# MisterPup/PDE-MultiGrid

Hardware: AMD Instinct MI355X
Metric: MLUPS on 3D Poisson 512^3 V-cycle (higher is better)
Workload: dtype f64

## Files before the change

include/mgx.h:

```cpp
#ifndef MGX_H
#define MGX_H

#include <stddef.h>
#include <stdint.h>

#ifdef __cplusplus
extern "C" {
#endif

typedef enum {
    MGX_OK = 0,
    MGX_ERR_INVALID = 1,
    MGX_ERR_SIZE = 2,
    MGX_ERR_HIP = 3,
    MGX_ERR_NOMEM = 4,
    MGX_ERR_RCCL = 5,
    MGX_ERR_NOGPU = 6
} mgx_status;

typedef enum { MGX_RESIDUAL_REF_COMPAT = 0, MGX_RESIDUAL_CORRECT = 1 } mgx_residual_mode;

typedef struct mgx_ctx mgx_ctx;
typedef struct mgx_event mgx_event;

// ... 6 lines not shown
int mgx_ctx_create(int device, mgx_ctx** out);
int mgx_ctx_destroy(mgx_ctx* ctx);
int mgx_ctx_sync(mgx_ctx* ctx);
int mgx_ctx_check(mgx_ctx* ctx);
int mgx_ctx_clear_abort(mgx_ctx* ctx, int reenable);
int mgx_ctx_generation(const mgx_ctx* ctx, unsigned long long* generation);
int mgx_ctx_prepare(mgx_ctx* ctx);
int mgx_ctx_device(const mgx_ctx* ctx, int* device);
int mgx_ctx_set_param(mgx_ctx* ctx, const char* name, int value);
const char* mgx_ctx_last_relax_kernel(const mgx_ctx* ctx);
const char* mgx_ctx_last_rr_kernel(const mgx_ctx* ctx);
const char* mgx_ctx_last_corr_kernel(const mgx_ctx* ctx);
const char* mgx_ctx_last_block3_kernel(const mgx_ctx* ctx);
int mgx3dxs_relax_block3_f64(mgx_ctx* ctx, const double* vin, double* vout, const double* f, const int n[3], const double h[3],
                             int first_colour, int store_both);
int mgx_test_set_lds_poison(int on);
int mgx_test_lds_probe(mgx_ctx* ctx, double* fraction);
int mgx_ctx_stream(const mgx_ctx* ctx, void** hip_stream);

int mgx_malloc(mgx_ctx* ctx, size_t bytes, void** dptr);
int mgx_free(mgx_ctx* ctx, void* dptr);
int mgx_memcpy_h2d(mgx_ctx* ctx, void* dst, const void* host_src, size_t bytes);
int mgx_memcpy_d2h(mgx_ctx* ctx, void* host_dst, const void* src, size_t bytes);
int mgx_memcpy_d2d(mgx_ctx* ctx, void* dst, const void* src, size_t bytes);
int mgx_memset_zero(mgx_ctx* ctx, void* dst, size_t bytes);

int mgx_graph_begin(mgx_ctx* ctx);
int mgx_graph_end(mgx_ctx* ctx, void** graph_exec);
int mgx_graph_launch(mgx_ctx* ctx, void* graph_exec);
int mgx_graph_destroy(mgx_ctx* ctx, void* graph_exec);
// ... 195 lines not shown
     \
     \
     \
     \
     \
     \
     \
     \
     \
     \
    int mgx3dxs_corr_fused_takes_##SFX(const mgx_ctx* ctx, const int n[3], int nplanes);                \
     \
     \
     \
    int mgx3dxs_block3_up_takes_##SFX(const mgx_ctx* ctx, const int n[3], int ncycles);                 \
    int mgx3dxs_correct_pset_slab_##SFX(mgx_ctx* ctx, real* v, const int n[3], int fzoff,               \
                                        const real* coarse_v, const int cn[3], int czoff, int zmin,     \
                                        int zmax);                                                      \
    int mgx3dxs_relax_corr_colour_slab_##SFX(mgx_ctx* ctx, real* v, const real* f, const int n[3],      \
                                             int fzoff, const real h[3], const real* coarse_v,          \
                                             const int cn[3], int czoff, int cplanes, int zbeg,         \
                                             int zend);                                                 \
     \
     \
     \
    int mgx3dxs_interpolate_correct_colour_##SFX(mgx_ctx* ctx, real* v, const int n[3],                 \
                                                 const real* coarse_v, const int cn[3], int colour);    \
    int mgx3dxs_interpolate_correct_colour_slab_##SFX(mgx_ctx* ctx, real* v, const int n[3], int fzoff, \
                                                      const real* coarse_v, const int cn[3], int czoff, \
                                                      int pzbeg, int pzend, int colour);                \
// ... 203 lines not shown
```

pde_multigrid_amd/csrc/host/mg_multigrid3d.inc:

```

#define GRID MG_CAT(mgGrid3D_, R)
#define MGRID MG_CAT(mgMultiGrid3D_, R)
#define FN(name) MG_CAT3(mgMultiGrid3D_, R, _##name)
#define MGXL(mg, name) ((mg)->layout ? MG_CAT3(mgx3dxs_, name##_, R) : MG_CAT3(mgx3d_, name##_, R))

static size_t MG_CAT(vol3_, R)(const GRID* g) { return (size_t)g->sizeX * g->sizeY * g->sizeZ; }
static size_t MG_CAT(dvol3_, R)(int layout, const GRID* g) {
    return layout ? MG_CAT(mgx3dxs_elems_, R)(g->sizeXYZ) : MG_CAT(vol3_, R)(g);
}

static int MG_CAT(grid3_new_, R)(mgx_ctx* ctx, int layout, const int sizeXYZ[3], const REAL range[6], GRID** out) {
    for (int d = 0; d < 3; d++)
        MG_REQUIRE(sizeXYZ[d] >= 3 && (sizeXYZ[d] - 1) % 2 == 0, MGX_ERR_SIZE, "Grid3D: size[%d] = %d is not odd and >= 3", d,
                   sizeXYZ[d]);
    MG_REQUIRE(range[1] > range[0] && range[3] > range[2] && range[5] > range[4], MGX_ERR_INVALID,
               "Grid3D: empty range");
    GRID* g = (GRID*)calloc(1, sizeof(GRID));
    MG_REQUIRE(g, MGX_ERR_NOMEM, "Grid3D: out of host memory");
    g->sizeX = g->sizeXYZ[0] = sizeXYZ[0];
    g->sizeY = g->sizeXYZ[1] = sizeXYZ[1];
    g->sizeZ = g->sizeXYZ[2] = sizeXYZ[2];
    REAL x_range = range[1] - range[0];
    REAL y_range = range[3] - range[2];
    REAL z_range = range[5] - range[4];
// ... 523 lines not shown
        if (down_done) {
        } else if (mg->fuse && mg->f_rim_zero[gridID + 1]) {
            MG_TRY(MGXL(mg, residual_restrict_keep_rim)(mg->ctx, fine->d_v, fine->d_f, fine->sizeXYZ, h, mg->residual_mode,
                                                        coarse->d_f, coarse->sizeXYZ));
        } else if (mg->fuse) {
            MG_TRY(MGXL(mg, residual_restrict)(mg->ctx, fine->d_v, fine->d_f, fine->sizeXYZ, h, mg->residual_mode, coarse->d_f,
                                          coarse->sizeXYZ));
            mg->f_rim_zero[gridID + 1] = 1;
        } else {
            REAL* residual = NULL;
            MG_TRY(FN(CalculateResidual)(mg, fine, &residual));
            MG_TRY(FN(Restrict)(mg, residual, fine->sizeXYZ, coarse->d_f, coarse->sizeXYZ));
        }
        MG_TRY(MG_CAT(vcycle_body3_, R)(mg, gridID + 1, v1, v2, 1));
        if (mg->fuse && mg->layout && mg->smoother == 0 && v2 > 0) {
            MG_TRY(MG_CAT(mgx3dxs_interpolate_correct_relax_pp_, R)(mg->ctx, fine->d_v, fine->d_e, fine->d_f, fine->sizeXYZ, h, coarse->d_v,
                                                                    coarse->sizeXYZ, v2, mg->e_rim_valid[gridID]));
            if (MG_CAT(mgx3dxs_relax_pp_takes_, R)(mg->ctx, fine->sizeXYZ, v2) && !MG_CAT(mgx3dxs_corr_fused_takes_, R)(mg->ctx, fine->sizeXYZ, fine->sizeZ - 2))
                mg->e_rim_valid[gridID] = 1;
            if (MG_CAT(mgx3dxs_block3_up_takes_, R)(mg->ctx, fine->sizeXYZ, v2))
                mg->e_rim_valid[gridID] = 1;
            return MGX_OK;
        } else if (mg->fuse) {
            MG_TRY(MGXL(mg, interpolate_correct)(mg->ctx, fine->d_v, fine->sizeXYZ, coarse->d_v, coarse->sizeXYZ));
        } else {
            MG_TRY(FN(Interpolate)(mg, fine->d_e, fine->sizeXYZ, coarse->d_v, coarse->sizeXYZ));
            MG_TRY(FN(ApplyCorrection)(mg, fine->d_v, fine->sizeXYZ, fine->d_e, fine->sizeXYZ));
        }
    }
    return FN(Relax)(mg, fine, v2);
// ... 370 lines not shown
```

pde_multigrid_amd/csrc/mgx_block3d.hip:

```cpp
#include <type_traits>

#include "mgx_internal.hpp"
#include "mgx_kernels3d.hpp"

namespace mgx {

template <class real, int COL, bool STORE_BOTH, int TW>
__global__ void __launch_bounds__(64 * TW, 4)
    relax3d_xs_block3_kernel(const real* vin, real* vout, const real* __restrict__ f, int sx, int sy, int sz, real hx2, real hy2,
                             real hz2, int zrun, int gx, int gy, int xcd_mode) {
    constexpr int ROWS = 2 * TW, OUTR = ROWS - 6;
    static_assert(OUTR % 2 == 0, "the colour parity of a wave's rows must not depend on the tile");
    __shared__ real sY[2][TW][2][64];
    __shared__ real sX[2][TW][2][64];
    __shared__ real sZ[2][TW][2][64];
    const Geo<XSplit, real> g(sx, sy);
    const int lane = threadIdx.x;
    const int w = __builtin_amdgcn_readfirstlane(threadIdx.y);
    int bx, by, bz;
    tile_of_block(xcd_mode, gx, gy, bx, by, bz);
    const int z0 = 1 + bz * zrun, z1 = min(z0 + zrun, sz - 1);
    if (z0 >= z1) return;
    const int PL = (int)g.PL;

    const int Hn = (sx + 1) >> 1;
    const int pn = bx * 60 + lane - 2, p = min(max(pn, 0), Hn - 1);
    const unsigned off0 = (unsigned)p * (unsigned)sizeof(real), off1 = (unsigned)(g.H + (p <= Hn - 2 ? p : 0)) * (unsigned)sizeof(real);
// ... 3 lines not shown
    const bool xface0 = pn <= 0 || pn >= Hn - 1;
    const bool wxface = bx * 60 - 2 <= 0 || bx * 60 + 61 >= Hn - 1;
    const bool outlane = lane >= 2 && lane <= 61;
    int roff[2];
    bool yin[2], outrow[2];
#pragma unroll
    for (int o = 0; o < 2; o++) {
        const int y = by * OUTR - 3 + 2 * w + o;
        roff[o] = min(max(y, 0), sy - 1) * g.P;
        yin[o] = y >= 1 && y <= sy - 2;
        outrow[o] = 2 * w + o >= 3 && 2 * w + o < ROWS - 3;
    }
    const int wU = w > 0 ? w - 1 : 0, wD = w < TW - 1 ? w + 1 : TW - 1;
    auto zc = [&](int z) { return min(max(z, 0), sz - 1); };
    auto plane = [&](const real* a, int z) { return plane_rsrc<real>(a + (ptrdiff_t)zc(z) * (ptrdiff_t)g.PL, PL, 1); };

    real a_m[2], a_c[2], a_p[2], a_n[2], fx_c[2], fx_1[2], fx_2[2], fx_n[2], xv_n[2], fy_c[2], fy_n[2];
    real b_c[2], b_m[2], b_mm[2], d_c[2], d_m[2], d_mm[2], x3[2];
#pragma unroll
    for (int o = 0; o < 2; o++)
        a_m[o] = a_c[o] = a_p[o] = a_n[o] = fx_c[o] = fx_1[o] = fx_2[o] = fx_n[o] = xv_n[o] = fy_c[o] = fy_n[o] = b_c[o] =
            b_m[o] = b_mm[o] = d_c[o] = d_m[o] = d_mm[o] = x3[o] = 0;

    const int t0 = z0 - 2, tlast = z1 + 1;
    {
        const auto qm = plane(vin, t0 - 1), q0 = plane(vin, t0), qp = plane(vin, t0 + 1);
        const bool zf = t0 <= 0 || t0 >= sz - 1;
        const auto qf = plane(f, t0);
#pragma unroll
        for (int o = 0; o < 2; o++) {
            const int hx = (COL + 1 + o + t0) & 1;
            a_m[o] = buf_load<real>(qm, off(hx), roff[o]);
            a_c[o] = buf_load<real>(q0, off(hx ^ 1), roff[o]);
            a_p[o] = buf_load<real>(qp, off(hx), roff[o]);
            fx_c[o] = buf_load<real>(zf || !yin[o] ? q0 : qf, off(hx), roff[o]);
            if (wxface) xv_n[o] = buf_load<real>(q0, off(0), roff[o]);
        }
        __builtin_amdgcn_s_waitcnt(0x0F70);
#pragma unroll
        for (int o = 0; o < 2; o++)
            if (wxface && ((COL + 1 + o + t0) & 1) == 0 && xface0) fx_c[o] = xv_n[o];
        const int b = (t0 - 1) & 1;
        sY[b][w][0][lane] = a_c[0];
        sY[b][w][1][lane] = a_c[1];
        asm volatile("s_waitcnt lgkmcnt(0)\n\ts_barrier" ::: "memory");
    }

    auto relax = [&](auto hc, int o, const real (&c)[2], real nb, real sb, real D, real U, real fv) __attribute__((always_inline)) {
        constexpr int h = decltype(hc)::value;
        real O, E;
        if (h == 0) {
            O = wave_from_prev_lane<real>(c[o]);
            E = c[o];
        } else {
            O = c[o];
            E = wave_from_next_lane<real>(c[o]);
// ... 8 lines not shown
        const auto ro3 = plane(vout, t - 3), ro2 = plane(vout, t - 2);
        const auto rY = plane(vin, t + 2), rXv = plane(vin, t + 1), rFx = plane(f, t + 1), rFy = plane(f, t);
        const bool zf = t + 1 <= 0 || t + 1 >= sz - 1;
        __builtin_amdgcn_s_setprio(3);
#pragma unroll
        for (int o = 0; o < 2; o++) {
            const int hx = (COL + 1 + o + PAR) & 1;
            const bool sto = outlane && yin[o] && outrow[o];
            if (t - 3 >= z0 && t - 3 < z1 && sto && xin(hx ^ 1)) buf_store_nt<real>(x3[o], ro3, off(hx ^ 1), roff[o]);
            if (STORE_BOTH && t - 2 >= z0 && t - 2 < z1 && sto && xin(hx ^ 1)) buf_store_nt<real>(d_m[o], ro2, off(hx ^ 1), roff[o]);
            a_n[o] = buf_load<real>(rY, off(hx ^ 1), roff[o]);
            fx_n[o] = buf_load<real>(zf || !yin[o] ? rXv : rFx, off(hx ^ 1), roff[o]);
            if ((hx ^ 1) == 0 && wxface) xv_n[o] = buf_load<real>(rXv, off(0), roff[o]);
            fy_n[o] = buf_load<real>(rFy, off(hx ^ 1), roff[o]);
        }
        __builtin_amdgcn_s_setprio(0);
        const bool zin1 = t >= 1 && t <= sz - 2, zin2 = t - 1 >= 1 && t - 1 <= sz - 2;
        {
            const real nb = sY[PB][wU][1][lane], sb = sY[PB][wD][0][lane];
#pragma unroll
            for (int o = 0; o < 2; o++) {
                const real v1 = (((COL + 1 + PAR) & 1) ^ o) == 0
                                    ? relax(std::integral_constant<int, 0>{}, o, a_c, nb, sb, a_m[o], a_p[o], fx_c[o])
                                    : relax(std::integral_constant<int, 1>{}, o, a_c, nb, sb, a_m[o], a_p[o], fx_c[o]);
                const int hx = (COL + 1 + o + PAR) & 1;
                b_c[o] = zin1 && yin[o] && xin(hx) ? v1 : fx_c[o];
            }
        }
        {
            const real nb = sX[PB][wU][1][lane], sb = sX[PB][wD][0][lane];
// ... 3 lines not shown
                                    ? relax(std::integral_constant<int, 0>{}, o, b_m, nb, sb, b_mm[o], b_c[o], fy_c[o])
                                    : relax(std::integral_constant<int, 1>{}, o, b_m, nb, sb, b_mm[o], b_c[o], fy_c[o]);
                const int hx = (COL + 1 + o + PAR) & 1;
                d_c[o] = zin2 && yin[o] && xin(hx) ? v2 : a_m[o];
            }
        }
        {
            const real nb = sZ[PB][wU][1][lane], sb = sZ[PB][wD][0][lane];
#pragma unroll
            for (int o = 0; o < 2; o++) {
                x3[o] = (((COL + 1 + PAR) & 1) ^ o) == 0
                            ? relax(std::integral_constant<int, 0>{}, o, d_m, nb, sb, d_mm[o], d_c[o], fx_2[o])
                            : relax(std::integral_constant<int, 1>{}, o, d_m, nb, sb, d_mm[o], d_c[o], fx_2[o]);
            }
        }
#pragma unroll
        for (int o = 0; o < 2; o++) {
            sY[PAR][w][o][lane] = a_p[o];
            sX[PAR][w][o][lane] = b_c[o];
            sZ[PAR][w][o][lane] = d_c[o];
        }
        asm volatile("s_waitcnt lgkmcnt(0)\n\ts_barrier" ::: "memory");
        __builtin_amdgcn_s_waitcnt(0x0F70);
#pragma unroll
        for (int o = 0; o < 2; o++) {
            a_m[o] = a_c[o]; a_c[o] = a_p[o]; a_p[o] = a_n[o];
            fx_2[o] = fx_1[o]; fx_1[o] = fx_c[o];
            fx_c[o] = ((COL + 1 + o + PAR) & 1) == 1 && wxface && xface0 ? xv_n[o] : fx_n[o];
            fy_c[o] = fy_n[o];
            b_mm[o] = b_m[o]; b_m[o] = b_c[o];
            d_mm[o] = d_m[o]; d_m[o] = d_c[o];
        }
    };

    int t = t0;
    if (t & 1) iteration(std::integral_constant<int, 1>{}, t++);
    for (;; t += 2) {
        iteration(std::integral_constant<int, 0>{}, t);
        if (t == tlast) break;
        iteration(std::integral_constant<int, 1>{}, t + 1);
        if (t + 1 == tlast) break;
// ... 4 lines not shown
        for (int o = 0; o < 2; o++) {
            const int hx = (COL + 1 + o + tlast) & 1;
            if (outlane && yin[o] && outrow[o] && xin(hx)) buf_store_nt<real>(x3[o], ro3, off(hx), roff[o]);
        }
    }
}

bool relax_block3_takes(const mgx_ctx* ctx, const int n[3], size_t elem, int part) {
    if (!(ctx->block3 & part) || elem != 8) return false;
    if ((unsigned long long)Geo<XSplit, double>(n[0], n[1]).PL * 8ull >= (1ull << 31)) return false;
    return n[0] >= 385 && n[1] >= 129 && n[2] >= 65;
}

template <class real>
void relax3d_xs_block3_launch(mgx_ctx* ctx, const real* vin, real* vout, const real* f, const int n[3], real hx2, real hy2, real hz2,
                              int first_colour, bool store_both) {
    constexpr int TW = 16;
    const int gx = ceil_div((n[0] - 1) / 2, 60), gy = ceil_div(n[1] - 2, 2 * TW - 6);
    const int tiles = gx * gy, planes = n[2] - 2;
    const int zrun = ceil_div(planes, runs_filling_rounds(tiles, planes, ctx->num_cus, 64, 16, 4));
    const dim3 grid(tiles * ceil_div(planes, zrun), 1, 1), blk(64, TW, 1);
#define MGX_B3(C, S)                                                                                                          \
    MGX_LAUNCH((relax3d_xs_block3_kernel<real, C, S, TW>), grid, blk, 0, ctx->compute, vin, vout, f, n[0], n[1], n[2], hx2, hy2, \
               hz2, zrun, gx, gy, 1)
    if (first_colour == 0) {
        if (store_both) MGX_B3(0, true); else MGX_B3(0, false);
    } else {
        if (store_both) MGX_B3(1, true); else MGX_B3(1, false);
    }
#undef MGX_B3
    snprintf(ctx->last_block3_kernel, sizeof ctx->last_block3_kernel, "relax3d_xs_block3_kernel<%s,%d,%s,%d>",
             sizeof(real) == 8 ? "double" : "float", first_colour, store_both ? "true" : "false", TW);
}
template void relax3d_xs_block3_launch<double>(mgx_ctx*, const double*, double*, const double*, const int[3], double, double, double, int,
                                               bool);

}

extern "C" int mgx3dxs_relax_block3_f64(mgx_ctx* ctx, const double* vin, double* vout, const double* f, const int n[3], const double h[3],
                                        int first_colour, int store_both) {
    MGX_REQUIRE(ctx && vin && vout && f && n && h, MGX_ERR_INVALID, "relax_block3: NULL argument");
    MGX_USE(ctx);
    MGX_REQUIRE(mgx::valid_size(n[0]) && mgx::valid_size(n[1]) && mgx::valid_size(n[2]), MGX_ERR_SIZE,
                "relax_block3: sizes %d x %d x %d are not odd and >= 3", n[0], n[1], n[2]);
    MGX_REQUIRE(first_colour == 0 || first_colour == 1, MGX_ERR_INVALID, "relax_block3: first_colour = %d not in {0, 1}", first_colour);
    const unsigned long long plane_bytes = (unsigned long long)mgx::Geo<mgx::XSplit, double>(n[0], n[1]).PL * 8ull;
    MGX_REQUIRE(plane_bytes < (1ull << 31), MGX_ERR_SIZE,
                "relax_block3: a plane of %d x %d is too large", n[0], n[1]);
    MGX_REQUIRE(!store_both || vin != vout, MGX_ERR_INVALID, "relax_block3: store_both needs vout != vin");
    mgx::relax3d_xs_block3_launch<double>(ctx, vin, vout, f, n, h[0] * h[0], h[1] * h[1], h[2] * h[2], first_colour, store_both != 0);
    MGX_LAUNCH_CHECK();
    return MGX_OK;
}
```

pde_multigrid_amd/csrc/mgx_internal.hpp:

```cpp
#pragma once
#include <hip/hip_runtime.h>

#include <cstdarg>
#include <cstdio>
#include <cstring>
#include <type_traits>

#include "mgx.h"

struct mgx_ctx {
    int device = 0;
    hipStream_t compute = nullptr;
    hipStream_t comm = nullptr;
    hipEvent_t ev_compute = nullptr;
    hipEvent_t ev_comm = nullptr;
    int comm_inline = 0;
    int relax_ty = 4;
    int relax_zchunk = 0;
    int relax_xcd = 1;
    int rr_rows = 0;
    int rr_rcp = 1;
    int mixed_fused = 0;
    int mixed_rows = 4;
    int mixed_zchunk = 0;
// ... 37 lines not shown
    size_t scratch_bytes = 0;
    void* rccl_comm = nullptr;
    void* local_group = nullptr;
    int rank = 0, nranks = 1;
    int comm_rehearse = 0;
    void* rehearse_buf = nullptr;
    size_t rehearse_bytes = 0;
    int num_cus = 256;
    int pipe_unroll = 7;
    int corr_low = 0;
    int slab_edges_merged = 1;
    int resident_tile = 0;
    char last_corr_kernel[96] = "";
    char last_rr_kernel[96] = "";
    char last_relax_kernel[96] = "";
    int block3 = 3;
    char last_block3_kernel[96] = "";
};

struct mgx_event {
    hipEvent_t ev = nullptr;
};

namespace mgx {

void set_error(const char* fmt, ...);

inline int fail(int status, const char* fmt, ...) {
    char buf[512];
    va_list ap;
    va_start(ap, fmt);
// ... 82 lines not shown
```

pde_multigrid_amd/csrc/mgx_kernels3d.hip:

```cpp
#include <type_traits>

#include "mgx_internal.hpp"
#include "mgx_kernels3d.hpp"
#include "mgx_sync.hpp"

namespace mgx {

template <class real>
__global__ void __launch_bounds__(256) relax3d_colour_kernel(real* __restrict__ v, const real* __restrict__ f, int sx,
                                                             int sy, int sz, real hx2, real hy2, real hz2, int colour) {
    const int y = 1 + blockIdx.y * blockDim.y + threadIdx.y;
    const int z = 1 + blockIdx.z;
    if (y >= sy - 1) return;
    const int p = (colour + y + z) & 1;
    const int x = 2 * (blockIdx.x * blockDim.x + threadIdx.x) + p;
    if (x < 1 || x >= sx - 1) return;
    const size_t sxy = (size_t)sx * sy;
    const size_t i = x + (size_t)y * sx + (size_t)z * sxy;
    const real O = v[i - 1], E = v[i + 1];
    const real N = v[i - sx], S = v[i + sx];
    const real D = v[i - sxy], U = v[i + sxy];
    v[i] = relax3d_point<real>(O, E, N, S, D, U, f[i], hx2, hy2, hz2);
}

// ... 2559 lines not shown

template <class real, class L>
int residual_restrict3d(mgx_ctx* ctx, const real* v, const real* f, const int n[3], const real h[3], int mode,
                        real* coarse_f, const int cn[3], bool rim_is_zero = false) {
    MGX_TRY_RET(check_rr_args(ctx, ctx && v && f && h && coarse_f, n, cn, "residual_restrict3d"));
    MGX_REQUIRE(mode == MGX_RESIDUAL_REF_COMPAT || mode == MGX_RESIDUAL_CORRECT, MGX_ERR_INVALID,
                "residual_restrict3d: bad mode %d", mode);
    return residual_restrict3d_range<real, L>(ctx, v, f, n, 0, h, mode, coarse_f, cn, 0, 0, cn[2], rim_is_zero);
}

bool relax_rr3d_xs_takes(const mgx_ctx* ctx, const int n[3], const int cn[3], size_t elem);

bool relax_block3_takes(const mgx_ctx* ctx, const int n[3], size_t elem, int part);
template <class real>
void relax3d_xs_block3_launch(mgx_ctx* ctx, const real* vin, real* vout, const real* f, const int n[3], real hx2, real hy2, real hz2,
                              int first_colour, bool store_both);
template <>
void relax3d_xs_block3_launch<float>(mgx_ctx*, const float*, float*, const float*, const int[3], float, float, float, int, bool) {}

template <class real>
int relax_rr3d_slab(mgx_ctx* ctx, real* v, const real* f, const int n[3], int fzoff, const real h[3], int mode, real* coarse_f,
                    const int cn[3], int czoff, int pzbeg, int pzend) {
    MGX_TRY_RET(check_rr_args(ctx, ctx && v && f && h && coarse_f, n, cn, "relax_rr_slab"));
    MGX_REQUIRE(mode == MGX_RESIDUAL_REF_COMPAT || mode == MGX_RESIDUAL_CORRECT, MGX_ERR_INVALID, "relax_rr_slab: bad mode %d", mode);
    MGX_REQUIRE(pzbeg >= 1 && pzend <= cn[2] - 1 && pzbeg < pzend && czoff >= 0 && czoff <= pzbeg && fzoff >= 0 && (fzoff & 1) == 0 &&
                    fzoff <= (2 * pzbeg - 3 > 0 ? 2 * pzbeg - 3 : 0),
                MGX_ERR_INVALID, "relax_rr_slab: coarse planes [%d, %d) with offsets %d / %d", pzbeg, pzend, fzoff, czoff);
    MGX_REQUIRE(relax_rr3d_xs_takes(ctx, n, cn, sizeof(real)), MGX_ERR_INVALID, "relax_rr_slab: the level is not taken (ask relax_rr_takes)");
    const Geo<XSplit, real> gc(cn[0], cn[1]);
    MGX_TRY_RET(fill_zero(ctx, coarse_f + gc.PL * (size_t)(pzbeg - czoff), gc.PL * (size_t)(pzend - pzbeg) * sizeof(real)));
    MGX_REQUIRE(relax_rr3d_xs_launch<real>(ctx, v, f, n, h, mode, coarse_f, cn, fzoff, czoff, pzbeg, pzend), MGX_ERR_INVALID,
                "relax_rr_slab: launch refused");
    MGX_LAUNCH_CHECK();
// ... 221 lines not shown
        pipe_launch<real, false, 2, 4, 2, 2>(ctx, p, v, vo, f, sx, sy, zb, ze, hx2, hy2, hz2, colour, coarse_sh, cx, cy, szl, ckmax, zg0);
    else
        pipe_launch<real, false, 2, 8, 2, 2>(ctx, p, v, vo, f, sx, sy, zb, ze, hx2, hy2, hz2, colour, coarse_sh, cx, cy, szl, ckmax, zg0);
    memcpy(ctx->last_corr_kernel, ctx->last_relax_kernel, sizeof ctx->last_corr_kernel);
}

template <class real>
int relax3d_xs_pp(mgx_ctx* ctx, real* v, real* w, const real* f, const int n[3], const real h[3], int ncycles, int w_rim_valid);
template <class real>
void copy_rim3d_xs(mgx_ctx* ctx, const real* v, real* w, const int n[3]);

static bool block3_up_takes(const mgx_ctx* ctx, const int n[3], size_t elem, int ncycles) {
    return ncycles >= 2 && corr_fused_takes(ctx, n[0], n[1], n[2], n[2] - 2) && relax_block3_takes(ctx, n, elem, 2);
}

template <class real>
int interpolate_correct_relax3d_xs(mgx_ctx* ctx, real* v, const real* f, const int n[3], const real h[3], const real* coarse_v,
                                   const int cn[3], int ncycles, real* w = nullptr, int w_rim_valid = 0) {
    MGX_REQUIRE(ctx && v && f && h && coarse_v, MGX_ERR_INVALID, "interpolate_correct_relax3d: NULL argument");
    MGX_USE(ctx);
    int st = check_n3(n, "interpolate_correct_relax3d");
    if (st) return st;
    st = check_coarse3(n, cn, "interpolate_correct_relax3d");
    if (st) return st;
    MGX_REQUIRE(ncycles >= 1, MGX_ERR_INVALID, "interpolate_correct_relax3d: ncycles = %d < 1 (use interpolate_correct)", ncycles);
    ctx->last_corr_kernel[0] = 0;
    ctx->last_block3_kernel[0] = 0;
    const real hx2 = h[0] * h[0], hy2 = h[1] * h[1], hz2 = h[2] * h[2];
    const int sx = n[0], sy = n[1], sz = n[2], zb = 1, ze = sz - 1;
    if (!corr_fused_takes(ctx, sx, sy, sz, ze - zb)) {
        st = interpolate_correct3d_slab<real>(ctx, v, n, 0, coarse_v, cn, 0, 0, cn[2] - 1, 1);
        if (st) return st;
        if (w) return relax3d_xs_pp<real>(ctx, v, w, f, n, h, ncycles, w_rim_valid);
// ... 296 lines not shown
                                                        coarse_f, cn, coarse_rim_is_zero);                       \
    }                                                                                                            \
    int mgx3dxs_relax_rr_takes_##SFX(const mgx_ctx* ctx, const int n[3], const int cn[3]) {                     \
        return ctx && n && cn && mgx::relax_rr3d_xs_takes(ctx, n, cn, sizeof(real));                             \
    }                                                                                                            \
    int mgx3dxs_relax_rr_slab_##SFX(mgx_ctx* ctx, real* v, const real* f, const int n[3], int fzoff,            \
                                    const real h[3], int mode, real* coarse_f, const int cn[3], int czoff,       \
                                    int pzbeg, int pzend) {                                                      \
        return mgx::relax_rr3d_slab<real>(ctx, v, f, n, fzoff, h, mode, coarse_f, cn, czoff, pzbeg, pzend);      \
    }                                                                                                            \
    int mgx3dxs_corr_fused_takes_##SFX(const mgx_ctx* ctx, const int n[3], int nplanes) {                        \
        return ctx && n && mgx::corr_fused_takes(ctx, n[0], n[1], n[2], nplanes);                                \
    }                                                                                                            \
    int mgx3dxs_block3_up_takes_##SFX(const mgx_ctx* ctx, const int n[3], int ncycles) {                         \
        return ctx && n && mgx::block3_up_takes(ctx, n, sizeof(real), ncycles);                                  \
    }                                                                                                            \
    int mgx3dxs_correct_pset_slab_##SFX(mgx_ctx* ctx, real* v, const int n[3], int fzoff, const real* coarse_v,  \
                                        const int cn[3], int czoff, int zmin, int zmax) {                        \
        return mgx::correct_pset3d_slab<real>(ctx, v, n, fzoff, coarse_v, cn, czoff, zmin, zmax);                \
    }                                                                                                            \
    int mgx3dxs_relax_corr_colour_slab_##SFX(mgx_ctx* ctx, real* v, const real* f, const int n[3], int fzoff,    \
                                             const real h[3], const real* coarse_v, const int cn[3], int czoff,  \
                                             int cplanes, int zbeg, int zend) {                                  \
        return mgx::relax3d_corr_colour_slab<real>(ctx, v, f, n, fzoff, h, coarse_v, cn, czoff, cplanes, zbeg,   \
                                                   zend);                                                        \
    }                                                                                                            \
    int mgx3dxs_interpolate_correct_relax_pp_##SFX(mgx_ctx* ctx, real* v, real* w, const real* f, const int n[3], \
                                                   const real h[3], const real* coarse_v, const int cn[3],       \
                                                   int ncycles, int w_rim_valid) {                               \
        if (!w) return mgx::fail(MGX_ERR_INVALID, "interpolate_correct_relax_pp: w is NULL");                    \
// ... 154 lines not shown
#else
        return mgx::fail(MGX_ERR_INVALID, "set_param: 'relax3d.fused_dbg' exists only in diagnostic builds (make diag)");
#endif
    } else if (!strcmp(name, "relax3d.fused_lead")) {
        MGX_REQUIRE(value == 0 || (value >= 5 && value <= 7), MGX_ERR_INVALID, "relax3d.fused_lead (planes the red stage runs ahead) must be 0 (default), 5, 6 or 7");
        ctx->sweep_lead = value;
    } else if (!strcmp(name, "relax3d.unroll")) {
        MGX_REQUIRE(value >= 0 && value <= 31, MGX_ERR_INVALID, "set_param: relax3d.unroll = %d not in [0, 31]", value);
        ctx->pipe_unroll = value;
    } else if (!strcmp(name, "relax3d.block3")) {
        MGX_REQUIRE(value == 0 || value == 1, MGX_ERR_INVALID, "set_param: relax3d.block3 = %d not in {0, 1}", value);
        ctx->block3 = (ctx->block3 & ~1) | value;
    } else if (!strcmp(name, "relax3d.block3_up")) {
        MGX_REQUIRE(value == 0 || value == 1, MGX_ERR_INVALID, "set_param: relax3d.block3_up = %d not in {0, 1}", value);
        ctx->block3 = (ctx->block3 & ~2) | (value << 1);
    } else if (!strcmp(name, "relax3d.zchunk")) {
        MGX_REQUIRE(value >= 0, MGX_ERR_INVALID, "relax3d.zchunk must be >= 0 (0 = automatic)");
        ctx->relax_zchunk = value;
    } else {
        return mgx::fail(MGX_ERR_INVALID, "set_param: unknown parameter '%s'", name);
    }
    return MGX_OK;
}
}
```

pde_multigrid_amd/multigrid.py:

```python
import ctypes as C

import numpy as np

from ._lib import CORRECT, REF_COMPAT, check, lib


def _ct(dtype):
    dtype = np.dtype(dtype)
    if dtype == np.float32:
        return "f32", C.c_float
    if dtype == np.float64:
        return "f64", C.c_double
    raise TypeError("dtype must be float32 or float64, got %s" % dtype)


def _ip(a):
    return (C.c_int * len(a))(*[int(x) for x in a])


def _rp(a, ct):
    return (ct * len(a))(*[float(x) for x in a])


def _shape(n):
# ... 262 lines not shown

    def sweep_once(self, ctx, vin, vout, f, n, rng, zero=False, dtype=None):
        dtype = dtype or vin.dtype
        fn, ct = self._fn("sweep_once", dtype)
        h = _rp(grid_spacing(n, rng, dtype), ct)
        return self._run(ctx, [vin, vout, f], lambda a, o, b: fn(ctx._h, a, o, b, _ip(n), h, C.c_int(int(zero))), 1, _shape(n), dtype)

    def relax_pp_takes(self, ctx, n, ncycles, dtype=np.float64):
        s, _ = _ct(dtype)
        return bool(getattr(lib, "mgx3dxs_relax_pp_takes_" + s)(ctx._h, _ip(n), C.c_int(ncycles)))

    def block3_up_takes(self, ctx, n, ncycles, dtype=np.float64):
        s, _ = _ct(dtype)
        return bool(getattr(lib, "mgx3dxs_block3_up_takes_" + s)(ctx._h, _ip(n), C.c_int(ncycles)))

    def residual(self, ctx, v, f, n, rng, mode=REF_COMPAT, dtype=None):
        dtype = dtype or v.dtype
        fn, ct = self._fn("residual", dtype)
        h = _rp(grid_spacing(n, rng, dtype), ct)
        r = np.zeros(_shape(n), dtype)
        return self._run(ctx, [v, f, r], lambda a, b, c: fn(ctx._h, a, b, c, _ip(n), h, C.c_int(mode)), 2, _shape(n), dtype)

    def residual_restrict(self, ctx, v, f, n, rng, mode=REF_COMPAT, dtype=None):
        dtype = dtype or v.dtype
        fn, ct = self._fn("residual_restrict", dtype)
        h = _rp(grid_spacing(n, rng, dtype), ct)
        cn = coarse_size(n)
        coarse = np.zeros(_shape(cn), dtype)
        return self._run(ctx, [v, f, coarse], lambda a, b, c: fn(ctx._h, a, b, _ip(n), h, C.c_int(mode), c, _ip(cn)), 2,
                         _shape(cn), dtype)
# ... 55 lines not shown
            out_v = xs_unpack(ctx.to_host(pv, tuple(_shape(n)[:-1]) + (xs_geometry(n[0], isz)[1],), dtype), n[0])
            out_c = xs_unpack(ctx.to_host(pc, tuple(_shape(cn)[:-1]) + (xs_geometry(cn[0], isz)[1],), dtype), cn[0])
            return out_v, out_c
        finally:
            for q in (pv, pf, pc):
                ctx.free(q)

    def relax_block3(self, ctx, vin, f, n, rng, first_colour=0, store_both=False, vout=None):
        h = _rp(grid_spacing(n, rng, np.float64), C.c_double)
        arrs = [vin, f] if vout is None else [vin, f, vout]
        if vout is None:
            call = lambda a, b: lib.mgx3dxs_relax_block3_f64(ctx._h, a, a, b, _ip(n), h, C.c_int(first_colour), C.c_int(int(store_both)))
            return self._run(ctx, arrs, call, 0, _shape(n), np.float64)
        call = lambda a, b, c: lib.mgx3dxs_relax_block3_f64(ctx._h, a, c, b, _ip(n), h, C.c_int(first_colour), C.c_int(int(store_both)))
        return self._run(ctx, arrs, call, 2, _shape(n), np.float64)

    def interpolate_correct_relax(self, ctx, v, f, n, rng, coarse, ncycles, dtype=None):
        dtype = dtype or v.dtype
        fn, ct = self._fn("interpolate_correct_relax", dtype)
        h = _rp(grid_spacing(n, rng, dtype), ct)
        cn = coarse_size(n)
        return self._run(ctx, [v, f, coarse], lambda a, b, c: fn(ctx._h, a, b, _ip(n), h, c, _ip(cn), C.c_int(ncycles)), 0, _shape(n),
                         dtype)

    def jacobi(self, ctx, v, f, n, rng, omega, ncycles, dtype=None):
        dtype = dtype or v.dtype
        fn, ct = self._fn("jacobi", dtype)
        h = _rp(grid_spacing(n, rng, dtype), ct)
        return self._run(ctx, [v, np.zeros_like(v), f], lambda a, t, b: fn(ctx._h, a, t, b, _ip(n), h, ct(omega), C.c_int(ncycles)),
                         0, _shape(n), dtype)
# ... 922 lines not shown
```

Before: 226,900.

## Fuse coarse-grid interpolation correction into the block3 three-colour relax kernel

Adds a CORR variant of the temporally blocked block3 relax kernel that streams coarse-grid planes, trilinearly interpolates the correction on the fly, and adds it to the fine values as they enter the register pipeline. The post-smoothing path then uses this kernel, followed by remaining single passes, instead of a separate interpolate-correct-relax sequence. The block3_corr bit is enabled by default. This removes a full pass over the fine grid for the correction. In exchange the kernel carries more registers and extra coarse loads, which may reduce occupancy.

```diff
diff --git a/include/mgx.h b/include/mgx.h
--- a/include/mgx.h
+++ b/include/mgx.h
@@ -44,6 +44,8 @@
 const char* mgx_ctx_last_block3_kernel(const mgx_ctx* ctx);
 int mgx3dxs_relax_block3_f64(mgx_ctx* ctx, const double* vin, double* vout, const double* f, const int n[3], const double h[3],
                              int first_colour, int store_both);
+int mgx3dxs_relax_block3_corr_f64(mgx_ctx* ctx, double* v, const double* f, const int n[3], const double h[3], const double* coarse_v,
+                                  const int cn[3]);
 int mgx_test_set_lds_poison(int on);
 int mgx_test_lds_probe(mgx_ctx* ctx, double* fraction);
 int mgx_ctx_stream(const mgx_ctx* ctx, void** hip_stream);
@@ -269,6 +271,15 @@
      \
      \
     int mgx3dxs_block3_up_takes_##SFX(const mgx_ctx* ctx, const int n[3], int ncycles);                 \
+     \
+     \
+     \
+     \
+    int mgx3dxs_block3_corr_takes_##SFX(const mgx_ctx* ctx, const int n[3], int ncycles);               \
+    int mgx3dxs_interpolate_correct_relax_block3_##SFX(mgx_ctx* ctx, real* v, const real* f,            \
+                                                       const int n[3], const real h[3],                 \
+                                                       const real* coarse_v, const int cn[3],           \
+                                                       int ncycles);                                    \
     int mgx3dxs_correct_pset_slab_##SFX(mgx_ctx* ctx, real* v, const int n[3], int fzoff,               \
                                         const real* coarse_v, const int cn[3], int czoff, int zmin,     \
                                         int zmax);                                                      \
diff --git a/pde_multigrid_amd/csrc/host/mg_multigrid3d.inc b/pde_multigrid_amd/csrc/host/mg_multigrid3d.inc
--- a/pde_multigrid_amd/csrc/host/mg_multigrid3d.inc
+++ b/pde_multigrid_amd/csrc/host/mg_multigrid3d.inc
@@ -561,6 +561,11 @@
         }
         MG_TRY(MG_CAT(vcycle_body3_, R)(mg, gridID + 1, v1, v2, 1));
         if (mg->fuse && mg->layout && mg->smoother == 0 && v2 > 0) {
+            if (MG_CAT(mgx3dxs_block3_corr_takes_, R)(mg->ctx, fine->sizeXYZ, v2)) {
+                MG_TRY(MG_CAT(mgx3dxs_interpolate_correct_relax_block3_, R)(mg->ctx, fine->d_v, fine->d_f, fine->sizeXYZ, h, coarse->d_v,
+                                                                            coarse->sizeXYZ, v2));
+                return MGX_OK;
+            }
             MG_TRY(MG_CAT(mgx3dxs_interpolate_correct_relax_pp_, R)(mg->ctx, fine->d_v, fine->d_e, fine->d_f, fine->sizeXYZ, h, coarse->d_v,
                                                                     coarse->sizeXYZ, v2, mg->e_rim_valid[gridID]));
             if (MG_CAT(mgx3dxs_relax_pp_takes_, R)(mg->ctx, fine->sizeXYZ, v2) && !MG_CAT(mgx3dxs_corr_fused_takes_, R)(mg->ctx, fine->sizeXYZ, fine->sizeZ - 2))
diff --git a/pde_multigrid_amd/csrc/mgx_block3d.hip b/pde_multigrid_amd/csrc/mgx_block3d.hip
--- a/pde_multigrid_amd/csrc/mgx_block3d.hip
+++ b/pde_multigrid_amd/csrc/mgx_block3d.hip
@@ -5,12 +5,14 @@
 
 namespace mgx {
 
-template <class real, int COL, bool STORE_BOTH, int TW>
+template <class real, int COL, bool STORE_BOTH, int TW, bool CORR = false>
 __global__ void __launch_bounds__(64 * TW, 4)
     relax3d_xs_block3_kernel(const real* vin, real* vout, const real* __restrict__ f, int sx, int sy, int sz, real hx2, real hy2,
-                             real hz2, int zrun, int gx, int gy, int xcd_mode) {
+                             real hz2, int zrun, int gx, int gy, int xcd_mode, const real* coarse = nullptr, int cx = 0,
+                             int cy = 0) {
     constexpr int ROWS = 2 * TW, OUTR = ROWS - 6;
     static_assert(OUTR % 2 == 0, "the colour parity of a wave's rows must not depend on the tile");
+    static_assert(!CORR || (COL == 0 && !STORE_BOTH), "the correcting variant is R', B, R with red stored");
     __shared__ real sY[2][TW][2][64];
     __shared__ real sX[2][TW][2][64];
     __shared__ real sZ[2][TW][2][64];
@@ -44,13 +46,29 @@
     const int wU = w > 0 ? w - 1 : 0, wD = w < TW - 1 ? w + 1 : TW - 1;
     auto zc = [&](int z) { return min(max(z, 0), sz - 1); };
     auto plane = [&](const real* a, int z) { return plane_rsrc<real>(a + (ptrdiff_t)zc(z) * (ptrdiff_t)g.PL, PL, 1); };
+    const Geo<XSplit, real> gc(CORR ? cx : 3, CORR ? cy : 3);
+    const int cz = (sz + 1) >> 1;
+    int croff[2];
+#pragma unroll
+    for (int i = 0; i < 2; i++) croff[i] = CORR ? min(max(by * (OUTR / 2) - 2 + w + i, 0), cy - 1) * gc.P : 0;
+    const unsigned coff = (unsigned)XSplit::pos(p, gc.H) * (unsigned)sizeof(real);
+    auto cplane = [&](int k) {
+        return plane_rsrc<real>(coarse + (ptrdiff_t)min(max(k, 0), cz - 1) * (ptrdiff_t)gc.PL, (int)gc.PL, 1);
+    };
+    auto interp = [&](int ox, int oz, int o, const real (&k0)[2], const real (&k1)[2]) __attribute__((always_inline)) {
+        return interpolate3d_point<real>(ox, 1 - o, oz, [&](int dx, int dy, int dz) __attribute__((always_inline)) {
+            const real c = o + dy ? (dz ? k1[1] : k0[1]) : (dz ? k1[0] : k0[0]);
+            return dx ? wave_from_next_lane<real>(c) : c;
+        });
+    };
 
     real a_m[2], a_c[2], a_p[2], a_n[2], fx_c[2], fx_1[2], fx_2[2], fx_n[2], xv_n[2], fy_c[2], fy_n[2];
     real b_c[2], b_m[2], b_mm[2], d_c[2], d_m[2], d_mm[2], x3[2];
+    real c_0[2], c_1[2], c_n[2], e_n[2];
 #pragma unroll
     for (int o = 0; o < 2; o++)
         a_m[o] = a_c[o] = a_p[o] = a_n[o] = fx_c[o] = fx_1[o] = fx_2[o] = fx_n[o] = xv_n[o] = fy_c[o] = fy_n[o] = b_c[o] =
-            b_m[o] = b_mm[o] = d_c[o] = d_m[o] = d_mm[o] = x3[o] = 0;
+            b_m[o] = b_mm[o] = d_c[o] = d_m[o] = d_mm[o] = x3[o] = c_0[o] = c_1[o] = c_n[o] = e_n[o] = 0;
 
     const int t0 = z0 - 2, tlast = z1 + 1;
     {
@@ -70,6 +88,36 @@
 #pragma unroll
         for (int o = 0; o < 2; o++)
             if (wxface && ((COL + 1 + o + t0) & 1) == 0 && xface0) fx_c[o] = xv_n[o];
+        if constexpr (CORR) {
+#pragma unroll
+            for (int d = -1; d <= 1; d++) {
+                const int z = t0 + d;
+                const auto k0q = cplane(z >> 1), k1q = cplane((z >> 1) + 1);
+                real k0[2], k1[2];
+#pragma unroll
+                for (int i = 0; i < 2; i++) {
+                    k0[i] = buf_load<real>(k0q, coff, croff[i]);
+                    k1[i] = buf_load<real>(k1q, coff, croff[i]);
+                }
+                const bool zin = z >= 1 && z <= sz - 2;
+#pragma unroll
+                for (int o = 0; o < 2; o++) {
+                    const int hb = (COL + o + z) & 1;
+                    const real e = interp(hb, z & 1, o, k0, k1);
+                    real& a = d < 0 ? a_m[o] : d == 0 ? a_c[o] : a_p[o];
+                    if (zin && yin[o] && xin(hb)) a = a + e;
+                }
+            }
+            const int K = (t0 + 2) >> 1;
+            const auto q0c = cplane(K), q1c = cplane(K + 1), qnc = cplane(K + 2);
+#pragma unroll
+            for (int i = 0; i < 2; i++) {
+                c_0[i] = buf_load<real>(q0c, coff, croff[i]);
+                c_1[i] = buf_load<real>(q1c, coff, croff[i]);
+                c_n[i] = buf_load<real>(qnc, coff, croff[i]);
+            }
+            __builtin_amdgcn_s_waitcnt(0x0F70);
+        }
         const int b = (t0 - 1) & 1;
         sY[b][w][0][lane] = a_c[0];
         sY[b][w][1][lane] = a_c[1];
@@ -108,6 +156,13 @@
             if ((hx ^ 1) == 0 && wxface) xv_n[o] = buf_load<real>(rXv, off(0), roff[o]);
             fy_n[o] = buf_load<real>(rFy, off(hx ^ 1), roff[o]);
         }
+        if constexpr (CORR && PAR == 0) {
+            const auto qnc = cplane((t >> 1) + 3);
+            __builtin_amdgcn_sched_barrier(0);
+#pragma unroll
+            for (int i = 0; i < 2; i++) c_n[i] = buf_load<real>(qnc, coff, croff[i]);
+            __builtin_amdgcn_sched_barrier(0);
+        }
         __builtin_amdgcn_s_setprio(0);
         const bool zin1 = t >= 1 && t <= sz - 2, zin2 = t - 1 >= 1 && t - 1 <= sz - 2;
         {
@@ -141,6 +196,10 @@
                             : relax(std::integral_constant<int, 1>{}, o, d_m, nb, sb, d_mm[o], d_c[o], fx_2[o]);
             }
         }
+        if constexpr (CORR) {
+#pragma unroll
+            for (int o = 0; o < 2; o++) e_n[o] = interp((COL + o + PAR) & 1, PAR, o, c_0, c_1);
+        }
 #pragma unroll
         for (int o = 0; o < 2; o++) {
             sY[PAR][w][o][lane] = a_p[o];
@@ -148,10 +207,14 @@
             sZ[PAR][w][o][lane] = d_c[o];
         }
         asm volatile("s_waitcnt lgkmcnt(0)\n\ts_barrier" ::: "memory");
-        __builtin_amdgcn_s_waitcnt(0x0F70);
-#pragma unroll
-        for (int o = 0; o < 2; o++) {
-            a_m[o] = a_c[o]; a_c[o] = a_p[o]; a_p[o] = a_n[o];
+        if constexpr (CORR && PAR == 0) __builtin_amdgcn_s_waitcnt(0x0F72);
+        else __builtin_amdgcn_s_waitcnt(0x0F70);
+        const bool zin3 = t + 2 >= 1 && t + 2 <= sz - 2;
+#pragma unroll
+        for (int o = 0; o < 2; o++) {
+            a_m[o] = a_c[o]; a_c[o] = a_p[o];
+            a_p[o] = CORR && zin3 && yin[o] && xin((COL + o + PAR) & 1) ? a_n[o] + e_n[o] : a_n[o];
+            if constexpr (CORR && PAR == 1) { c_0[o] = c_1[o]; c_1[o] = c_n[o]; }
             fx_2[o] = fx_1[o]; fx_1[o] = fx_c[o];
             fx_c[o] = ((COL + 1 + o + PAR) & 1) == 1 && wxface && xface0 ? xv_n[o] : fx_n[o];
             fy_c[o] = fy_n[o];
@@ -186,7 +249,7 @@
 
 template <class real>
 void relax3d_xs_block3_launch(mgx_ctx* ctx, const real* vin, real* vout, const real* f, const int n[3], real hx2, real hy2, real hz2,
-                              int first_colour, bool store_both) {
+                              int first_colour, bool store_both, const real* coarse, const int* cn) {
     constexpr int TW = 16;
     const int gx = ceil_div((n[0] - 1) / 2, 60), gy = ceil_div(n[1] - 2, 2 * TW - 6);
     const int tiles = gx * gy, planes = n[2] - 2;
@@ -195,17 +258,20 @@
 #define MGX_B3(C, S)                                                                                                          \
     MGX_LAUNCH((relax3d_xs_block3_kernel<real, C, S, TW>), grid, blk, 0, ctx->compute, vin, vout, f, n[0], n[1], n[2], hx2, hy2, \
                hz2, zrun, gx, gy, 1)
-    if (first_colour == 0) {
+    if (coarse) {
+        MGX_LAUNCH((relax3d_xs_block3_kernel<real, 0, false, TW, true>), grid, blk, 0, ctx->compute, vin, vout, f, n[0], n[1], n[2], hx2,
+                   hy2, hz2, zrun, gx, gy, 1, coarse, cn[0], cn[1]);
+    } else if (first_colour == 0) {
         if (store_both) MGX_B3(0, true); else MGX_B3(0, false);
     } else {
         if (store_both) MGX_B3(1, true); else MGX_B3(1, false);
     }
 #undef MGX_B3
-    snprintf(ctx->last_block3_kernel, sizeof ctx->last_block3_kernel, "relax3d_xs_block3_kernel<%s,%d,%s,%d>",
-             sizeof(real) == 8 ? "double" : "float", first_colour, store_both ? "true" : "false", TW);
+    snprintf(ctx->last_block3_kernel, sizeof ctx->last_block3_kernel, "relax3d_xs_block3_kernel<%s,%d,%s,%d%s>",
+             sizeof(real) == 8 ? "double" : "float", first_colour, store_both ? "true" : "false", TW, coarse ? ",corr" : "");
 }
 template void relax3d_xs_block3_launch<double>(mgx_ctx*, const double*, double*, const double*, const int[3], double, double, double, int,
-                                               bool);
+                                               bool, const double*, const int*);
 
 }
 
@@ -220,7 +286,22 @@
     MGX_REQUIRE(plane_bytes < (1ull << 31), MGX_ERR_SIZE,
                 "relax_block3: a plane of %d x %d is too large", n[0], n[1]);
     MGX_REQUIRE(!store_both || vin != vout, MGX_ERR_INVALID, "relax_block3: store_both needs vout != vin");
-    mgx::relax3d_xs_block3_launch<double>(ctx, vin, vout, f, n, h[0] * h[0], h[1] * h[1], h[2] * h[2], first_colour, store_both != 0);
+    mgx::relax3d_xs_block3_launch<double>(ctx, vin, vout, f, n, h[0] * h[0], h[1] * h[1], h[2] * h[2], first_colour, store_both != 0, nullptr, nullptr);
     MGX_LAUNCH_CHECK();
     return MGX_OK;
 }
+
+extern "C" int mgx3dxs_relax_block3_corr_f64(mgx_ctx* ctx, double* v, const double* f, const int n[3], const double h[3], const double* coarse_v,
+                                             const int cn[3]) {
+    MGX_REQUIRE(ctx && v && f && n && h && coarse_v && cn, MGX_ERR_INVALID, "relax_block3_corr: NULL argument");
+    MGX_USE(ctx);
+    MGX_REQUIRE(mgx::valid_size(n[0]) && mgx::valid_size(n[1]) && mgx::valid_size(n[2]), MGX_ERR_SIZE,
+                "relax_block3_corr: sizes %d x %d x %d are not odd and >= 3", n[0], n[1], n[2]);
+    for (int d = 0; d < 3; d++)
+        MGX_REQUIRE(cn[d] == (n[d] - 1) / 2 + 1, MGX_ERR_SIZE, "relax_block3_corr: coarse size[%d] = %d != (%d-1)/2+1", d, cn[d], n[d]);
+    const unsigned long long plane_bytes = (unsigned long long)mgx::Geo<mgx::XSplit, double>(n[0], n[1]).PL * 8ull;
+    MGX_REQUIRE(plane_bytes < (1ull << 31), MGX_ERR_SIZE, "relax_block3_corr: a plane of %d x %d is too large", n[0], n[1]);
+    mgx::relax3d_xs_block3_launch<double>(ctx, v, v, f, n, h[0] * h[0], h[1] * h[1], h[2] * h[2], 0, false, coarse_v, cn);
+    MGX_LAUNCH_CHECK();
+    return MGX_OK;
+}
diff --git a/pde_multigrid_amd/csrc/mgx_internal.hpp b/pde_multigrid_amd/csrc/mgx_internal.hpp
--- a/pde_multigrid_amd/csrc/mgx_internal.hpp
+++ b/pde_multigrid_amd/csrc/mgx_internal.hpp
@@ -75,7 +75,7 @@
     char last_corr_kernel[96] = "";
     char last_rr_kernel[96] = "";
     char last_relax_kernel[96] = "";
-    int block3 = 3;
+    int block3 = 7;
     char last_block3_kernel[96] = "";
 };
 
diff --git a/pde_multigrid_amd/csrc/mgx_kernels3d.hip b/pde_multigrid_amd/csrc/mgx_kernels3d.hip
--- a/pde_multigrid_amd/csrc/mgx_kernels3d.hip
+++ b/pde_multigrid_amd/csrc/mgx_kernels3d.hip
@@ -2597,9 +2597,10 @@
 bool relax_block3_takes(const mgx_ctx* ctx, const int n[3], size_t elem, int part);
 template <class real>
 void relax3d_xs_block3_launch(mgx_ctx* ctx, const real* vin, real* vout, const real* f, const int n[3], real hx2, real hy2, real hz2,
-                              int first_colour, bool store_both);
+                              int first_colour, bool store_both, const real* coarse = nullptr, const int* cn = nullptr);
 template <>
-void relax3d_xs_block3_launch<float>(mgx_ctx*, const float*, float*, const float*, const int[3], float, float, float, int, bool) {}
+void relax3d_xs_block3_launch<float>(mgx_ctx*, const float*, float*, const float*, const int[3], float, float, float, int, bool, const float*,
+                                     const int*) {}
 
 template <class real>
 int relax_rr3d_slab(mgx_ctx* ctx, real* v, const real* f, const int n[3], int fzoff, const real h[3], int mode, real* coarse_f,
@@ -2851,9 +2852,35 @@
     return ncycles >= 2 && corr_fused_takes(ctx, n[0], n[1], n[2], n[2] - 2) && relax_block3_takes(ctx, n, elem, 2);
 }
 
+static bool block3_corr_takes(const mgx_ctx* ctx, const int n[3], size_t elem, int ncycles) {
+    return ncycles >= 2 && corr_fused_takes(ctx, n[0], n[1], n[2], n[2] - 2) && relax_block3_takes(ctx, n, elem, 4);
+}
+
 template <class real>
 int interpolate_correct_relax3d_xs(mgx_ctx* ctx, real* v, const real* f, const int n[3], const real h[3], const real* coarse_v,
-                                   const int cn[3], int ncycles, real* w = nullptr, int w_rim_valid = 0) {
+                                   const int cn[3], int ncycles, real* w = nullptr, int w_rim_valid = 0);
+template <class real>
+int interpolate_correct_relax_block3_xs(mgx_ctx* ctx, real* v, const real* f, const int n[3], const real h[3], const real* coarse_v,
+                                        const int cn[3], int ncycles) {
+    MGX_REQUIRE(ctx && v && f && h && coarse_v, MGX_ERR_INVALID, "interpolate_correct_relax_block3: NULL argument");
+    MGX_USE(ctx);
+    int st = check_n3(n, "interpolate_correct_relax_block3");
+    if (st) return st;
+    st = check_coarse3(n, cn, "interpolate_correct_relax_block3");
+    if (st) return st;
+    MGX_REQUIRE(ncycles >= 1, MGX_ERR_INVALID, "interpolate_correct_relax_block3: ncycles = %d < 1", ncycles);
+    if (!block3_corr_takes(ctx, n, sizeof(real), ncycles)) return interpolate_correct_relax3d_xs<real>(ctx, v, f, n, h, coarse_v, cn, ncycles, nullptr, 0);
+    ctx->last_corr_kernel[0] = 0;
+    const real hx2 = h[0] * h[0], hy2 = h[1] * h[1], hz2 = h[2] * h[2];
+    relax3d_xs_block3_launch<real>(ctx, v, v, f, n, hx2, hy2, hz2, 0, false, coarse_v, cn);
+    for (int s = 3; s < 2 * ncycles; s++) relax3d_xs_pass<real>(ctx, v, f, n[0], n[1], 1, n[2] - 1, hx2, hy2, hz2, s & 1);
+    MGX_LAUNCH_CHECK();
+    return MGX_OK;
+}
+
+template <class real>
+int interpolate_correct_relax3d_xs(mgx_ctx* ctx, real* v, const real* f, const int n[3], const real h[3], const real* coarse_v,
+                                   const int cn[3], int ncycles, real* w, int w_rim_valid) {
     MGX_REQUIRE(ctx && v && f && h && coarse_v, MGX_ERR_INVALID, "interpolate_correct_relax3d: NULL argument");
     MGX_USE(ctx);
     int st = check_n3(n, "interpolate_correct_relax3d");
@@ -3180,6 +3207,14 @@
     }                                                                                                            \
     int mgx3dxs_block3_up_takes_##SFX(const mgx_ctx* ctx, const int n[3], int ncycles) {                         \
         return ctx && n && mgx::block3_up_takes(ctx, n, sizeof(real), ncycles);                                  \
+    }                                                                                                            \
+    int mgx3dxs_block3_corr_takes_##SFX(const mgx_ctx* ctx, const int n[3], int ncycles) {                       \
+        return ctx && n && mgx::block3_corr_takes(ctx, n, sizeof(real), ncycles);                                \
+    }                                                                                                            \
+    int mgx3dxs_interpolate_correct_relax_block3_##SFX(mgx_ctx* ctx, real* v, const real* f, const int n[3],     \
+                                                       const real h[3], const real* coarse_v, const int cn[3],   \
+                                                       int ncycles) {                                            \
+        return mgx::interpolate_correct_relax_block3_xs<real>(ctx, v, f, n, h, coarse_v, cn, ncycles);           \
     }                                                                                                            \
     int mgx3dxs_correct_pset_slab_##SFX(mgx_ctx* ctx, real* v, const int n[3], int fzoff, const real* coarse_v,  \
                                         const int cn[3], int czoff, int zmin, int zmax) {                        \
@@ -3364,6 +3399,9 @@
     } else if (!strcmp(name, "relax3d.block3_up")) {
         MGX_REQUIRE(value == 0 || value == 1, MGX_ERR_INVALID, "set_param: relax3d.block3_up = %d not in {0, 1}", value);
         ctx->block3 = (ctx->block3 & ~2) | (value << 1);
+    } else if (!strcmp(name, "relax3d.block3_corr")) {
+        MGX_REQUIRE(value == 0 || value == 1, MGX_ERR_INVALID, "set_param: relax3d.block3_corr = %d not in {0, 1}", value);
+        ctx->block3 = (ctx->block3 & ~4) | (value << 2);
     } else if (!strcmp(name, "relax3d.zchunk")) {
         MGX_REQUIRE(value >= 0, MGX_ERR_INVALID, "relax3d.zchunk must be >= 0 (0 = automatic)");
         ctx->relax_zchunk = value;
diff --git a/pde_multigrid_amd/multigrid.py b/pde_multigrid_amd/multigrid.py
--- a/pde_multigrid_amd/multigrid.py
+++ b/pde_multigrid_amd/multigrid.py
@@ -300,6 +300,10 @@
         s, _ = _ct(dtype)
         return bool(getattr(lib, "mgx3dxs_block3_up_takes_" + s)(ctx._h, _ip(n), C.c_int(ncycles)))
 
+    def block3_corr_takes(self, ctx, n, ncycles, dtype=np.float64):
+        s, _ = _ct(dtype)
+        return bool(getattr(lib, "mgx3dxs_block3_corr_takes_" + s)(ctx._h, _ip(n), C.c_int(ncycles)))
+
     def residual(self, ctx, v, f, n, rng, mode=REF_COMPAT, dtype=None):
         dtype = dtype or v.dtype
         fn, ct = self._fn("residual", dtype)
@@ -385,6 +389,20 @@
             return self._run(ctx, arrs, call, 0, _shape(n), np.float64)
         call = lambda a, b, c: lib.mgx3dxs_relax_block3_f64(ctx._h, a, c, b, _ip(n), h, C.c_int(first_colour), C.c_int(int(store_both)))
         return self._run(ctx, arrs, call, 2, _shape(n), np.float64)
+
+    def relax_block3_corr(self, ctx, v, f, n, rng, coarse):
+        h = _rp(grid_spacing(n, rng, np.float64), C.c_double)
+        cn = coarse_size(n)
+        return self._run(ctx, [v, f, coarse], lambda a, b, c: lib.mgx3dxs_relax_block3_corr_f64(ctx._h, a, b, _ip(n), h, c, _ip(cn)), 0,
+                         _shape(n), np.float64)
+
+    def interpolate_correct_relax_block3(self, ctx, v, f, n, rng, coarse, ncycles, dtype=None):
+        dtype = dtype or v.dtype
+        fn, ct = self._fn("interpolate_correct_relax_block3", dtype)
+        h = _rp(grid_spacing(n, rng, dtype), ct)
+        cn = coarse_size(n)
+        return self._run(ctx, [v, f, coarse], lambda a, b, c: fn(ctx._h, a, b, _ip(n), h, c, _ip(cn), C.c_int(ncycles)), 0, _shape(n),
+                         dtype)
 
     def interpolate_correct_relax(self, ctx, v, f, n, rng, coarse, ncycles, dtype=None):
         dtype = dtype or v.dtype
```

Result: faster. 239,700 (median of 6 runs) (+5.7%).
